# ilovin/lstm_ctc_ocr

Hardware: AMD Instinct MI355X
Metric: captcha images/sec training (32x256, bs=64/GPU) (higher is better)
Workload: dtype bf16; 1 GPU; VGG-7 + BiLSTM(256) + CTC train step, H=32 W=256, 10-char labels, C=64, bs=64/GPU (BASELINE.json configs[1]), Adam lr 1e-4 wd 1e-5 clip 10; global_batch=64, parallelism=dp1, hipgraph=True

## Files before the change

### lstm_ctc_ocr_amd/csrc/common.h

```cpp
#pragma once
#include <stdlib.h>
#include <hip/hip_runtime.h>
#include <stdint.h>
#include <atomic>

#define OCR_WAVE 64

enum {
    OCR_OK = 0,
    OCR_ERR_MEMOPS = 1,
    OCR_ERR_INVALID = 2,
    OCR_ERR_EXEC = 3,
};

#define OCR_CHECK_LAUNCH()                                        \
    do {                                                          \
        hipError_t e__ = hipGetLastError();                       \
        if (e__ != hipSuccess) return OCR_ERR_EXEC;               \
    } while (0)

typedef uint16_t bf16_t;
typedef __attribute__((ext_vector_type(8))) __bf16 bf16x8;
typedef __attribute__((ext_vector_type(4))) float f32x4;
typedef __attribute__((ext_vector_type(4))) unsigned int u32x4;
// ... 3 lines not shown
    uint32_t u = __float_as_uint(f);
    if ((u & 0x7fffffffu) > 0x7f800000u) return (bf16_t)((u >> 16) | 0x40);
    u += 0x7fffu + ((u >> 16) & 1u);
    return (bf16_t)(u >> 16);
}
__device__ __forceinline__ float bf2f(bf16_t h) { return __uint_as_float(((uint32_t)h) << 16); }
typedef __attribute__((ext_vector_type(2))) __bf16 bf16x2_t;
__device__ __forceinline__ uint32_t pack_bf2(float lo, float hi) {
    bf16x2_t v = {(__bf16)lo, (__bf16)hi};
    return __builtin_bit_cast(uint32_t, v);
}
__device__ __forceinline__ float bf_lo(uint32_t p) { return __uint_as_float(p << 16); }
__device__ __forceinline__ float bf_hi(uint32_t p) { return __uint_as_float(p & 0xffff0000u); }

template <int CNT>
__device__ __forceinline__ uint32_t pool_code_word(const u32x4 (&rows)[CNT]) {
    uint32_t word = 0;
#pragma unroll
    for (int c = 0; c < 8; ++c) {
        float v[CNT];
#pragma unroll
        for (int e = 0; e < CNT; ++e) {
            const uint32_t pr = c < 2 ? rows[e].x : c < 4 ? rows[e].y : c < 6 ? rows[e].z : rows[e].w;
            v[e] = (c & 1) ? bf_hi(pr) : bf_lo(pr);
        }
        int best = 0; float bv = v[0];
#pragma unroll
        for (int e = 1; e < CNT; ++e) if (v[e] > bv) { bv = v[e]; best = e; }
        word |= (uint32_t)(best | ((bv > 0.f) ? 4 : 0)) << (4 * c);
    }
    return word;
}

__device__ __forceinline__ float wave_sum(float v) {
#pragma unroll
    for (int o = 32; o > 0; o >>= 1) v += __shfl_xor(v, o, 64);
    return v;
}
__device__ __forceinline__ float wave_max(float v) {
#pragma unroll
    for (int o = 32; o > 0; o >>= 1) v = fmaxf(v, __shfl_xor(v, o, 64));
    return v;
}

__device__ __forceinline__ float sigmoidf_(float x) { return __frcp_rn(1.0f + __expf(-x)); }
__device__ __forceinline__ float tanhf_(float x) {
    float e = __expf(-2.0f * fabsf(x));
    float t = (1.0f - e) * __frcp_rn(1.0f + e);
    return copysignf(t, x);
}

static inline const char* ocr_tune_env(const char* name) {
#ifdef OCR_EXPERIMENTS
    return getenv(name);
#else
    (void)name; return nullptr;
#endif
}
__device__ __forceinline__ long long ocr_wall_clock() { return (long long)__builtin_amdgcn_s_memrealtime(); }
__device__ __forceinline__ void ocr_clk_enter(long long* clk) {
    clk[0] = (long long)__builtin_amdgcn_s_memtime(); clk[1] = ocr_wall_clock();
}
__device__ __forceinline__ void ocr_clk_exit(long long* clk) {
    const long long c = (long long)__builtin_amdgcn_s_memtime(), t = ocr_wall_clock();
    clk[2] = c; clk[3] = t;
    clk[4] += c - clk[0]; clk[5] += t - clk[1]; clk[6] += 1;
// ... 17 lines not shown
```

### lstm_ctc_ocr_amd/csrc/conv_ws.hip

```cpp
#include "conv_plan.h"
#include <type_traits>

enum { WS_BIAS = 1, WS_RELU = 2, WS_MASK = 16, WS_ACCUM = 64 };

struct WsArgs {
    const bf16_t* P; const bf16_t* Q;
    int M, N, C, cW, cH;
    bf16_t* out; const float* bias; const bf16_t* mask; int flags;
    bf16_t* pool; int pool_kind;
    int ntiles, slots, per_slot, xcd_map;
    uint32_t* codes;
};

typedef __attribute__((address_space(3))) void* ws_lptr_t;
#define WS_OOB 0x80000000u

__device__ long long* g_ws_dbg;
extern "C" int ocr_conv_ws_debug(void* dbg) {
    long long* q = (long long*)dbg;
    return hipMemcpyToSymbol(HIP_SYMBOL(g_ws_dbg), &q, sizeof(q)) == hipSuccess ? OCR_OK : OCR_ERR_MEMOPS;
}
#define WS_PHASE(slot) do { if (wsdbg && tid == 0 && (slot) < 64) wsdbg[blockIdx.x * 64 + (slot)] = ocr_wall_clock(); } while (0)
__device__ long long* g_ws_clk;
int ws_set_clock_debug(void* dbg) {
    long long* p = (long long*)dbg;
    return hipMemcpyToSymbol(HIP_SYMBOL(g_ws_clk), &p, sizeof(p)) == hipSuccess ? OCR_OK : OCR_ERR_EXEC;
}

typedef short ws_s16x2 __attribute__((ext_vector_type(2)));
__device__ __forceinline__ uint32_t ws_max2(uint32_t a, uint32_t b) {
    return __builtin_bit_cast(uint32_t, __builtin_elementwise_max(__builtin_bit_cast(ws_s16x2, a), __builtin_bit_cast(ws_s16x2, b)));
}
__device__ __forceinline__ u32x4 ws_max8(u32x4 a, u32x4 b) {
    u32x4 r = {ws_max2(a.x, b.x), ws_max2(a.y, b.y), ws_max2(a.z, b.z), ws_max2(a.w, b.w)};
    return r;
}

typedef unsigned short ws_u16x2 __attribute__((ext_vector_type(2)));
template <int CNT>
__device__ __forceinline__ uint32_t ws_code2(const uint32_t (&p)[CNT]) {
    const ws_u16x2 one = {1, 1};
    ws_u16x2 v[CNT];
#pragma unroll
    for (int e = 0; e < CNT; ++e) v[e] = __builtin_bit_cast(ws_u16x2, p[e]);
    ws_u16x2 m = v[0];
#pragma unroll
    for (int e = 1; e < CNT; ++e) m = __builtin_elementwise_max(m, v[e]);
    ws_u16x2 t = __builtin_elementwise_min((ws_u16x2)(m - v[CNT - 2]), one);
#pragma unroll
    for (int e = CNT - 3; e >= 0; --e) t = __builtin_elementwise_min((ws_u16x2)(m - v[e]), one) * (ws_u16x2)(t + one);
    const ws_u16x2 code = t + (ws_u16x2)(__builtin_elementwise_min(m, one) << (ws_u16x2){2, 2});
    return __builtin_bit_cast(uint32_t, code);
}
template <int CNT>
__device__ __forceinline__ uint32_t ws_code_word(const u32x4 (&p)[CNT]) {
    uint32_t x[CNT], y[CNT], z[CNT], w[CNT];
#pragma unroll
    for (int e = 0; e < CNT; ++e) { x[e] = p[e].x; y[e] = p[e].y; z[e] = p[e].z; w[e] = p[e].w; }
    const uint32_t c0 = ws_code2(x), c1 = ws_code2(y), c2 = ws_code2(z), c3 = ws_code2(w);
    return ((c0 | (c0 >> 12)) & 0xffu) | (((c1 | (c1 >> 12)) & 0xffu) << 8) | (((c2 | (c2 >> 12)) & 0xffu) << 16) | ((c3 | (c3 >> 12)) << 24);
}

template <int H, int NC, int KSPLIT>
struct WsCfg {
    static constexpr int BM = NC * H;
    static constexpr int PG = 4 / KSPLIT;
    static constexpr int CF = NC < 16 ? NC : 16;
    static constexpr int HF = 16 / CF;
    static constexpr int HW = 4 * HF;
    static constexpr int PS = NC + 2;
    static constexpr int CHB = (H + 2) * PS * 128;
    static constexpr int BUFB = KSPLIT * CHB;
    static constexpr int PPC = H * PS / 8;
    static constexpr int PI = KSPLIT * PPC / 4;
    static constexpr int NFE = 4 / KSPLIT;
    static constexpr int HWE = NFE * HF;
    static constexpr int NPE = NC * HWE;
    static constexpr int XOFF = 2 * BUFB;
    static constexpr int SOFF = XOFF + (KSPLIT == 2 ? 4 * 8192 : 0);
    static constexpr int STW = NPE * 128;
    static constexpr int TOFF = SOFF + 4 * STW;
    static constexpr int BOFF = TOFF + 4 * PI * 128;
    static constexpr int MOFF = BOFF + 256;
    static constexpr int LDS_PLAIN = MOFF, LDS_MASK = MOFF + 4 * STW;
    static_assert(((NC + 1) * H + H) * 128 * 2 / 16 * 4 < 65536, "table entries fit 16 bits");
    static_assert(NC == CF && PG * HW == H && (H * PS) % 8 == 0 && (KSPLIT * PPC) % 4 == 0 && LDS_MASK <= 163840, "geometry");
    static_assert(((H + 1) * PS) * 128 < 65536, "ds_read immediates");
};

template <int H, int NC, int KSPLIT, bool MASK ,
          bool CODES = false >
__global__ __launch_bounds__(256) __attribute__((amdgpu_waves_per_eu(1, 1))) void conv_ws_kernel(WsArgs g) {
    using G = WsCfg<H, NC, KSPLIT>;
// ... 325 lines not shown
```

### lstm_ctc_ocr_amd/csrc/nn_ops.hip

```cpp
#include "common.h"
#include <stdlib.h>

__device__ __forceinline__ void unpack8(u32x4 p, float* f) {
    f[0] = bf_lo(p.x); f[1] = bf_hi(p.x); f[2] = bf_lo(p.y); f[3] = bf_hi(p.y);
    f[4] = bf_lo(p.z); f[5] = bf_hi(p.z); f[6] = bf_lo(p.w); f[7] = bf_hi(p.w);
}

__global__ __launch_bounds__(256) void conv1_fwd_kernel(const float* __restrict__ x,
                                                        const float* __restrict__ w,
                                                        const float* __restrict__ bias,
                                                        bf16_t* __restrict__ y, int Nb, int W, int H,
                                                        int Cout, int relu) {
    const int groups = Cout >> 3;
    const int gq = threadIdx.x % groups;
    const int plane = threadIdx.x / groups;
    const int planes = 256 / groups;
    float wr[9][8], br[8];
#pragma unroll
    for (int t = 0; t < 9; ++t)
#pragma unroll
        for (int c = 0; c < 8; ++c) wr[t][c] = w[t * Cout + gq * 8 + c];
#pragma unroll
    for (int c = 0; c < 8; ++c) br[c] = bias[gq * 8 + c];
    const long npix = (long)Nb * W * H;
    for (long pix = (long)blockIdx.x * planes + plane; pix < npix; pix += (long)gridDim.x * planes) {
        int h = (int)(pix % H);
        long q = pix / H;
        int wq = (int)(q % W);
        const float* xn = x + (q - wq) * H;
        float xv[9];
#pragma unroll
        for (int t = 0; t < 9; ++t) {
            int ww = wq + t / 3 - 1, hh = h + t % 3 - 1;
            xv[t] = ((unsigned)ww < (unsigned)W && (unsigned)hh < (unsigned)H) ? xn[(long)ww * H + hh] : 0.f;
// ... 42 lines not shown
#pragma unroll
            for (int c = 0; c < 8; ++c) acc[t][c] = fmaf(xv, dv[c], acc[t][c]);
        }
#pragma unroll
        for (int c = 0; c < 8; ++c) acc[9][c] += dv[c];
    }
    __shared__ float red[4][10][64];
#pragma unroll
    for (int t = 0; t < 10; ++t)
#pragma unroll
        for (int c = 0; c < 8; ++c) {
            float v = acc[t][c];
            v += __shfl_xor(v, 8, 64);
            v += __shfl_xor(v, 16, 64);
            v += __shfl_xor(v, 32, 64);
            acc[t][c] = v;
        }
    const int lane = threadIdx.x & 63, wave = threadIdx.x >> 6;
    if (lane < 8) {
#pragma unroll
        for (int t = 0; t < 10; ++t)
#pragma unroll
            for (int c = 0; c < 8; ++c) red[wave][t][lane * 8 + c] = acc[t][c];
    }
    __syncthreads();
    for (int i = threadIdx.x; i < 10 * 64; i += 256) {
        int t = i / 64, c = i % 64;
        float v = red[0][t][c] + red[1][t][c] + red[2][t][c] + red[3][t][c];
        if (t < 9) atomicAdd(dw + t * Cout + c, v);
        else atomicAdd(db + c, v);
    }
}

__device__ __forceinline__ void conv1_patch(const float* __restrict__ xn, int W, int H, int w0, int h0, float (&patch)[4][4]) {
#pragma unroll
    for (int i = 0; i < 4; ++i)
#pragma unroll
        for (int j = 0; j < 4; ++j) {
            const int ww = w0 - 1 + i, hh = h0 - 1 + j;
            patch[i][j] = ((unsigned)ww < (unsigned)W && (unsigned)hh < (unsigned)H) ? xn[(long)ww * H + hh] : 0.f;
        }
}
__device__ __forceinline__ int conv1_pool_code(float o0, float o1, float o2, float o3) {
    const float r[4] = {bf_lo(pack_bf2(o0, 0.f)), bf_lo(pack_bf2(o1, 0.f)), bf_lo(pack_bf2(o2, 0.f)), bf_lo(pack_bf2(o3, 0.f))};
    int best = 0; float bvv = r[0];
#pragma unroll
    for (int e = 1; e < 4; ++e) if (r[e] > bvv) { bvv = r[e]; best = e; }
    return best | ((bvv > 0.f) ? 4 : 0);
}
__device__ __forceinline__ void conv1_window(const float* __restrict__ xn, int W, int H, int w0, int h0,
                                             const float (&wr)[9][8], const float (&br)[8], float (&o)[4][8], float (&patch)[4][4]) {
    conv1_patch(xn, W, H, w0, h0, patch);
    typedef float f32x2 __attribute__((ext_vector_type(2)));
#pragma unroll
    for (int e = 0; e < 4; ++e) {
        const int a = e >> 1, b = e & 1;
        f32x2 acc2[4];
#pragma unroll
        for (int q = 0; q < 4; ++q) acc2[q] = (f32x2){0.f, 0.f};
#pragma unroll
        for (int t = 0; t < 9; ++t) {
            const float pv = patch[a + t / 3][b + t % 3];
#pragma unroll
            for (int q = 0; q < 4; ++q)
                acc2[q] = __builtin_elementwise_fma((f32x2){pv, pv}, (f32x2){wr[t][2 * q], wr[t][2 * q + 1]}, acc2[q]);
        }
#pragma unroll
        for (int q = 0; q < 4; ++q) {
            o[e][2 * q] = fmaxf(acc2[q].x + br[2 * q], 0.f);
            o[e][2 * q + 1] = fmaxf(acc2[q].y + br[2 * q + 1], 0.f);
        }
    }
}

#ifdef OCR_EXPERIMENTS
struct Conv1Patch { float v[4][4]; };
struct Conv1Raw { float t[4][4]; unsigned ok; };
__device__ __forceinline__ void conv1_patch_load(const float* __restrict__ x, int W, int H, int Wo, int Ho, unsigned op, Conv1Raw& raw) {
    const unsigned ho = op % (unsigned)Ho, q = op / (unsigned)Ho;
    const unsigned wo = q % (unsigned)Wo, n = q / (unsigned)Wo;
    const float* xn = x + (long)n * W * H;
    const int w0 = (int)wo * 2, h0 = (int)ho * 2;
    const bool r0 = w0 > 0, r3 = w0 + 2 < W, c0 = h0 > 0, c3 = h0 + 2 < H;
    const int wi[4] = {r0 ? w0 - 1 : 0, w0, w0 + 1, r3 ? w0 + 2 : w0 + 1};
    const int hj[4] = {c0 ? h0 - 1 : 0, h0, h0 + 1, c3 ? h0 + 2 : h0 + 1};
#pragma unroll
    for (int i = 0; i < 4; ++i)
#pragma unroll
        for (int j = 0; j < 4; ++j) raw.t[i][j] = xn[wi[i] * H + hj[j]];
    raw.ok = (r0 ? 1u : 0u) | (r3 ? 2u : 0u) | (c0 ? 4u : 0u) | (c3 ? 8u : 0u);
}
__device__ __forceinline__ void conv1_patch_select(const Conv1Raw& raw, Conv1Patch& pt) {
    const bool r0 = raw.ok & 1u, r3 = raw.ok & 2u, c0 = raw.ok & 4u, c3 = raw.ok & 8u;
#pragma unroll
    for (int i = 0; i < 4; ++i)
#pragma unroll
        for (int j = 0; j < 4; ++j) {
            const bool ok = (i != 0 || r0) && (i != 3 || r3) && (j != 0 || c0) && (j != 3 || c3);
            pt.v[i][j] = ok ? raw.t[i][j] : 0.f;
        }
}
__device__ __forceinline__ void conv1_pin_weights(float (&wr)[9][8], float (&br)[8]) {
#pragma unroll
    for (int t = 0; t < 9; ++t)
#pragma unroll
        for (int c = 0; c < 8; ++c) asm volatile("" : "+v"(wr[t][c]));
// ... 103 lines not shown
                const float xv = (a == 0) ? ((b == 0) ? cur.v[i][j] : cur.v[i][j + 1]) : ((b == 0) ? cur.v[i + 1][j] : cur.v[i + 1][j + 1]);
                acc[t][c] = fmaf(xv, gv, acc[t][c]);
            }
        }
    }
    __shared__ float red[4][10][64];
#pragma unroll
    for (int t = 0; t < 10; ++t)
#pragma unroll
        for (int c = 0; c < 8; ++c) {
            float v = acc[t][c];
            v += __shfl_xor(v, 8, 64);
            v += __shfl_xor(v, 16, 64);
            v += __shfl_xor(v, 32, 64);
            acc[t][c] = v;
        }
    const int lane = threadIdx.x & 63, wave = threadIdx.x >> 6;
    if (lane < 8) {
#pragma unroll
        for (int t = 0; t < 10; ++t)
#pragma unroll
            for (int c = 0; c < 8; ++c) red[wave][t][lane * 8 + c] = acc[t][c];
    }
    __syncthreads();
    for (int i = threadIdx.x; i < 10 * 64; i += 256) {
        int t = i / 64, c = i % 64;
        float v = red[0][t][c] + red[1][t][c] + red[2][t][c] + red[3][t][c];
        if (t < 9) atomicAdd(dw + t * Cout + c, v);
        else atomicAdd(db + c, v);
    }
}
#endif

template <bool CODES>
__device__ __forceinline__ void conv1_pool_fwd_body(const float* __restrict__ x, const float* __restrict__ w,
                                                    const float* __restrict__ bias, bf16_t* __restrict__ p,
                                                    int Nb, int W, int H, int Cout, f32x4* __restrict__ zero, long zero_n4,
                                                    uint32_t* __restrict__ codes, u32x4* __restrict__ ones, long ones_n4) {
    for (long i = (long)blockIdx.x * 256 + threadIdx.x; i < zero_n4; i += (long)gridDim.x * 256) zero[i] = (f32x4){0.f, 0.f, 0.f, 0.f};
    for (long i = (long)blockIdx.x * 256 + threadIdx.x; i < ones_n4; i += (long)gridDim.x * 256) ones[i] = (u32x4){~0u, ~0u, ~0u, ~0u};
    const int groups = Cout >> 3, gq = threadIdx.x % groups, plane = threadIdx.x / groups, planes = 256 / groups;
    float wr[9][8], br[8];
#pragma unroll
    for (int t = 0; t < 9; ++t)
#pragma unroll
        for (int c = 0; c < 8; ++c) wr[t][c] = w[t * Cout + gq * 8 + c];
#pragma unroll
    for (int c = 0; c < 8; ++c) br[c] = bias[gq * 8 + c];
    const int Wo = W >> 1, Ho = H >> 1;
    const long npix = (long)Nb * Wo * Ho;
    for (long op = (long)blockIdx.x * planes + plane; op < npix; op += (long)gridDim.x * planes) {
        const int ho = (int)(op % Ho);
        const long q = op / Ho;
        const int wo = (int)(q % Wo);
        const long n = q / Wo;
        float o[4][8], patch[4][4];
        conv1_window(x + n * W * H, W, H, wo * 2, ho * 2, wr, br, o, patch);
        float m[8];
#pragma unroll
        for (int c = 0; c < 8; ++c) m[c] = fmaxf(fmaxf(o[0][c], o[1][c]), fmaxf(o[2][c], o[3][c]));
        u32x4 pk = {pack_bf2(m[0], m[1]), pack_bf2(m[2], m[3]), pack_bf2(m[4], m[5]), pack_bf2(m[6], m[7])};
        *(u32x4*)(p + op * Cout + gq * 8) = pk;
        if constexpr (CODES) {
            uint32_t word = 0;
#pragma unroll
            for (int c = 0; c < 8; ++c) word |= (uint32_t)conv1_pool_code(o[0][c], o[1][c], o[2][c], o[3][c]) << (4 * c);
// ... 63 lines not shown
            acc[9][c] += gv;
            const float* px = mypatch + (best >> 1) * 4 + (best & 1);
#pragma unroll
            for (int t = 0; t < 9; ++t) acc[t][c] = fmaf(px[(t / 3) * 4 + t % 3], gv, acc[t][c]);
        }
    }
    __shared__ float red[4][10][64];
#pragma unroll
    for (int t = 0; t < 10; ++t)
#pragma unroll
        for (int c = 0; c < 8; ++c) {
            float v = acc[t][c];
            v += __shfl_xor(v, 8, 64);
            v += __shfl_xor(v, 16, 64);
            v += __shfl_xor(v, 32, 64);
            acc[t][c] = v;
        }
    const int lane = threadIdx.x & 63, wave = threadIdx.x >> 6;
    if (lane < 8) {
#pragma unroll
        for (int t = 0; t < 10; ++t)
#pragma unroll
            for (int c = 0; c < 8; ++c) red[wave][t][lane * 8 + c] = acc[t][c];
    }
    __syncthreads();
    for (int i = threadIdx.x; i < 10 * 64; i += 256) {
        int t = i / 64, c = i % 64;
        float v = red[0][t][c] + red[1][t][c] + red[2][t][c] + red[3][t][c];
        if (slab != nullptr) slab[(long)blockIdx.x * 640 + i] = v;
        else if (t < 9) atomicAdd(dw + t * Cout + c, v);
        else atomicAdd(db + c, v);
    }
}

__device__ __forceinline__ uint32_t max2(uint32_t a, uint32_t b) {
    uint32_t lo = (bf_lo(b) > bf_lo(a)) ? (b & 0xffffu) : (a & 0xffffu);
    uint32_t hi = (bf_hi(b) > bf_hi(a)) ? (b & 0xffff0000u) : (a & 0xffff0000u);
    return lo | hi;
}
__device__ __forceinline__ u32x4 max8(u32x4 a, u32x4 b) {
    u32x4 r = {max2(a.x, b.x), max2(a.y, b.y), max2(a.z, b.z), max2(a.w, b.w)};
    return r;
}

template <int KW, int KH>
__global__ __launch_bounds__(256) void maxpool_fwd_kernel(const bf16_t* __restrict__ x, bf16_t* __restrict__ y,
                                                          int Nb, int W, int H, int C) {
    constexpr int kw = KW, kh = KH;
    const int Wo = W / kw, Ho = H / kh, groups = C >> 3;
    const long total = (long)Nb * Wo * Ho * groups;
    for (long idx = (long)blockIdx.x * 256 + threadIdx.x; idx < total; idx += (long)gridDim.x * 256) {
        int gq = (int)(idx % groups);
        long op = idx / groups;
        int ho = (int)(op % Ho);
        long q = op / Ho;
        int wo = (int)(q % Wo);
        long n = q / Wo;
        const bf16_t* base = x + (((n * W + (long)wo * kw) * H) + (long)ho * kh) * C + gq * 8;
        u32x4 m = *(const u32x4*)base;
#pragma unroll
        for (int a = 0; a < kw; ++a)
#pragma unroll
            for (int b = 0; b < kh; ++b) {
                if (a == 0 && b == 0) continue;
                m = max8(m, *(const u32x4*)(base + ((long)a * H + b) * C));
            }
// ... 772 lines not shown
            const int g = (int)(i / U), u = (int)(i % U);
            out[(u >> 4) * 64 + g * 16 + (u & 15)] = jb.src[i];
        }
    } else {
        for (long i = ((long)b * 256 + threadIdx.x) * 4; i + 3 < jb.n; i += (long)jb.nblocks * 256 * 4) {
            f32x4 v = *(const f32x4*)(jb.src + i);
            u32x2 pk = {pack_bf2(v.x, v.y), pack_bf2(v.z, v.w)};
            *(u32x2*)(jb.dst + i) = pk;
        }
    }
}

__global__ __launch_bounds__(256) void eltwise_bf16_kernel(int op, const bf16_t* __restrict__ a, const bf16_t* __restrict__ b,
                                                           bf16_t* __restrict__ out, long n8) {
    for (long i = (long)blockIdx.x * 256 + threadIdx.x; i < n8; i += (long)gridDim.x * 256) {
        float x[8], y[8], o[8], z[8];
        unpack8(*(const u32x4*)(a + i * 8), x);
        if (op != 1) unpack8(*(const u32x4*)(b + i * 8), y);
        if (op == 4) unpack8(*(const u32x4*)(out + i * 8), z);
#pragma unroll
        for (int c = 0; c < 8; ++c) {
            if (op == 0) o[c] = x[c] + y[c];
            else if (op == 1) o[c] = fmaxf(x[c], 0.f);
            else if (op == 2) o[c] = y[c] > 0.f ? x[c] : 0.f;
            else if (op == 3) o[c] = fmaxf(x[c] + y[c], 0.f);
            else o[c] = z[c] + (y[c] > 0.f ? x[c] : 0.f);
        }
        u32x4 pk = {pack_bf2(o[0], o[1]), pack_bf2(o[2], o[3]), pack_bf2(o[4], o[5]), pack_bf2(o[6], o[7])};
        *(u32x4*)(out + i * 8) = pk;
    }
}

static bool nn_knob(const char* name, int slot) {
    static int v[2] = {-1, -1};
    if (v[slot] < 0) { const char* e = ocr_tune_env(name); v[slot] = (e && atoi(e) != 0) ? 1 : 0; }
    return v[slot] == 1;
}
#ifdef OCR_EXPERIMENTS
static bool conv1_v1() { return !nn_knob("OCR_CONV1_V2", 0); }
#endif
static bool col2im_v1() { return nn_knob("OCR_COL2IM_V1", 1); }
static inline int grid_for(long total, int cap = 4096) {
    long b = (total + 255) / 256;
    if (b > cap) b = cap;
    if (b < 1) b = 1;
    return (int)b;
}

extern "C" int ocr_conv1_fwd(const float* x, const float* w, const float* bias, void* y, int Nb, int W, int H,
                             int Cout, int relu, void* stream) {
    if (!x || !w || !bias || !y || (Cout & 7) || Cout > 1024) return OCR_ERR_INVALID;
    if (256 % (Cout >> 3)) return OCR_ERR_INVALID;
    long total = (long)Nb * W * H * (Cout >> 3);
    conv1_fwd_kernel<<<grid_for(total, 2048), 256, 0, (hipStream_t)stream>>>(
        x, w, bias, (bf16_t*)y, Nb, W, H, Cout, relu);
    OCR_CHECK_LAUNCH();
    return OCR_OK;
}
extern "C" int ocr_conv1_wgrad(const float* x, const void* dz, float* dw, float* db, int Nb, int W, int H, int Cout,
                               void* stream) {
    if (!x || !dz || !dw || !db || Cout != 64) return OCR_ERR_INVALID;
    long npix = (long)Nb * W * H;
    int ppb = 1024;
    conv1_wgrad_kernel<<<ceil_div(npix, ppb), 256, 0, (hipStream_t)stream>>>(x, (const bf16_t*)dz, dw, db, Nb, W, H, Cout, ppb);
    OCR_CHECK_LAUNCH();
    return OCR_OK;
}
extern "C" int ocr_eltwise_bf16(int op, const void* a, const void* b, void* out, long n, void* stream) {
    if (!a || !out || (op != 1 && !b) || op < 0 || op > 4 || n <= 0 || (n & 7)) return OCR_ERR_INVALID;
    eltwise_bf16_kernel<<<grid_for(n / 8, 4096), 256, 0, (hipStream_t)stream>>>(op, (const bf16_t*)a, (const bf16_t*)b, (bf16_t*)out, n / 8);
    OCR_CHECK_LAUNCH();
    return OCR_OK;
}
static int conv1_pool_fwd_impl(const float* x, const float* w, const float* bias, void* p, int Nb, int W, int H, int Cout,
                               float* zero, long zero_n, void* codes, void* ones, long ones_n, void* stream) {
    if (!x || !w || !bias || !p || (Cout & 7) || Cout > 1024 || 256 % (Cout >> 3) || (W & 1) || (H & 1)) return OCR_ERR_INVALID;
    if (zero_n < 0 || (zero_n & 3) || (zero_n && (!zero || ((size_t)zero & 15)))) return OCR_ERR_INVALID;
    if (ones_n < 0 || (ones_n & 3) || (ones_n && (!ones || ((size_t)ones & 15)))) return OCR_ERR_INVALID;
    if (codes && (Cout != 64 || ((size_t)codes & 3))) return OCR_ERR_INVALID;
    long total = (long)Nb * (W / 2) * (H / 2) * (Cout >> 3);
#ifdef OCR_EXPERIMENTS
    if (!zero_n && !ones_n && !codes && !conv1_v1() && (long)Nb * (W / 2) * (H / 2) < 0x7fffffffL && (long)Nb * W * H < 0x7fffffffL && (long)W * H < 0x7fffffffL)
        conv1_pool_fwd2_kernel<<<grid_for(total, 2048), 256, 0, (hipStream_t)stream>>>(x, w, bias, (bf16_t*)p, Nb, W, H, Cout);
    else
#endif
    {
        if (codes) conv1_pool_fwd_kernel<true><<<grid_for(total, 2048), 256, 0, (hipStream_t)stream>>>(x, w, bias, (bf16_t*)p, Nb, W, H, Cout, (f32x4*)zero,
                                                                                                          zero_n / 4, (uint32_t*)codes, (u32x4*)ones, ones_n / 4);
        else conv1_pool_fwd_kernel<false><<<grid_for(total, 2048), 256, 0, (hipStream_t)stream>>>(x, w, bias, (bf16_t*)p, Nb, W, H, Cout, (f32x4*)zero,
                                                                                                 zero_n / 4, nullptr, (u32x4*)ones, ones_n / 4);
    }
    OCR_CHECK_LAUNCH();
    return OCR_OK;
}
extern "C" int ocr_conv1_pool_fwd(const float* x, const float* w, const float* bias, void* p, int Nb, int W, int H, int Cout,
                                  void* stream) {
    return conv1_pool_fwd_impl(x, w, bias, p, Nb, W, H, Cout, nullptr, 0, nullptr, nullptr, 0, stream);
}
extern "C" int ocr_conv1_pool_fwd_train(const float* x, const float* w, const float* bias, void* p, int Nb, int W, int H, int Cout,
                                        void* codes, float* zero, long zero_n, void* ones, long ones_n, void* stream) {
    return conv1_pool_fwd_impl(x, w, bias, p, Nb, W, H, Cout, zero, zero_n, codes, ones, ones_n, stream);
}
static int conv1_ppb() {
    static int v = -1;
    if (v < 0) { const char* e = getenv("OCR_CONV1_PPB"); v = e ? atoi(e) : 256; if (v < 32 || v > 1024 || (v & 31)) v = 256; }
    return v;
}
static int conv1_pool_bwd_impl(const float* x, const float* w, const float* bias, const void* dp, float* dw, float* db,
                               int Nb, int W, int H, int Cout, const void* codes, float* slab, void* stream) {
    if (!x || !w || !bias || !dp || (!slab && (!dw || !db)) || Cout != 64 || (W & 1) || (H & 1) || ((size_t)codes & 3)) return OCR_ERR_INVALID;
    long npix = (long)Nb * (W / 2) * (H / 2);
    int ppb = slab ? conv1_ppb() : 256;
#ifdef OCR_EXPERIMENTS
    if (!codes && !slab && !conv1_v1() && npix < 0x7fffffffL - 512 && (long)Nb * W * H < 0x7fffffffL)
        conv1_pool_bwd2_kernel<<<ceil_div(npix, ppb), 256, 0, (hipStream_t)stream>>>(x, w, bias, (const bf16_t*)dp, dw, db, Nb, W, H,
                                                                                     Cout, ppb);
    else
#endif
    {
        if (codes) conv1_pool_bwd_kernel<true><<<ceil_div(npix, ppb), 256, 0, (hipStream_t)stream>>>(x, w, bias, (const bf16_t*)dp, dw, db, Nb, W, H,
                                                                                                   Cout, ppb, (const uint32_t*)codes, slab);
        else conv1_pool_bwd_kernel<false><<<ceil_div(npix, ppb), 256, 0, (hipStream_t)stream>>>(x, w, bias, (const bf16_t*)dp, dw, db, Nb, W, H,
                                                                                               Cout, ppb, nullptr, slab);
    }
    OCR_CHECK_LAUNCH();
    return OCR_OK;
}
extern "C" int ocr_conv1_pool_bwd(const float* x, const float* w, const float* bias, const void* dp, float* dw, float* db,
                                  int Nb, int W, int H, int Cout, void* stream) {
    return conv1_pool_bwd_impl(x, w, bias, dp, dw, db, Nb, W, H, Cout, nullptr, nullptr, stream);
}
extern "C" int ocr_conv1_pool_bwd_codes(const float* x, const float* w, const float* bias, const void* dp, float* dw, float* db,
                                        int Nb, int W, int H, int Cout, const void* codes, void* stream) {
    if (!codes) return OCR_ERR_INVALID;
    return conv1_pool_bwd_impl(x, w, bias, dp, dw, db, Nb, W, H, Cout, codes, nullptr, stream);
}
extern "C" int ocr_conv1_pool_bwd_slab_rows(int Nb, int W, int H) {
    if (Nb <= 0 || W <= 0 || H <= 0 || (W & 1) || (H & 1)) return 0;
    return (int)ceil_div((long)Nb * (W / 2) * (H / 2), (long)conv1_ppb());
}
extern "C" int ocr_conv1_pool_bwd_slab(const float* x, const float* w, const float* bias, const void* dp, int Nb, int W, int H, int Cout,
                                       const void* codes, float* slab, void* stream) {
    if (!slab || ((size_t)slab & 15)) return OCR_ERR_INVALID;
    return conv1_pool_bwd_impl(x, w, bias, dp, nullptr, nullptr, Nb, W, H, Cout, codes, slab, stream);
}
extern "C" int ocr_maxpool_fwd(const void* x, void* y, int Nb, int W, int H, int C, int kw, int kh, void* stream) {
    if (!x || !y || (C & 7) || kw < 1 || kw > 2 || kh < 1 || kh > 2 || W % kw || H % kh) return OCR_ERR_INVALID;
    long total = (long)Nb * (W / kw) * (H / kh) * (C >> 3);
    const bf16_t* xi = (const bf16_t*)x; bf16_t* yo = (bf16_t*)y;
    hipStream_t st = (hipStream_t)stream;
    int gr = grid_for(total, 8192);
    if (kw == 2 && kh == 2) maxpool_fwd_kernel<2, 2><<<gr, 256, 0, st>>>(xi, yo, Nb, W, H, C);
    else if (kw == 1 && kh == 2) maxpool_fwd_kernel<1, 2><<<gr, 256, 0, st>>>(xi, yo, Nb, W, H, C);
    else if (kw == 2 && kh == 1) maxpool_fwd_kernel<2, 1><<<gr, 256, 0, st>>>(xi, yo, Nb, W, H, C);
    else return OCR_ERR_INVALID;
    OCR_CHECK_LAUNCH();
    return OCR_OK;
// ... 272 lines not shown
```

Before: 56360 images/sec.

## Stage conv1 input rows in LDS tiles for fused conv+pool forward and backward

Replaces the default conv1+maxpool forward and backward kernels with tile kernels. Each block stages the contiguous span of input rows it needs into shared memory, with zero padding, then computes per-pixel 3x3 windows from LDS instead of global loads. Index divisions are replaced by precomputed reciprocal multiplies. The forward pass packs bf16 outputs and pool codes with a shared u16 max/code helper, and the old kernels stay reachable only under experiment knobs. This trades global-memory traffic for dynamic LDS allocation that may limit occupancy, and adds new geometry checks that return an error on large shapes.

```diff
diff --git a/lstm_ctc_ocr_amd/csrc/common.h b/lstm_ctc_ocr_amd/csrc/common.h
--- a/lstm_ctc_ocr_amd/csrc/common.h
+++ b/lstm_ctc_ocr_amd/csrc/common.h
@@ -59,6 +59,27 @@
     return word;
 }
 
+typedef unsigned short u16x2_t __attribute__((ext_vector_type(2)));
+template <int CNT>
+__device__ __forceinline__ uint32_t pool_code2_u16(const uint32_t (&p)[CNT], uint32_t& mx) {
+    const u16x2_t one = {1, 1};
+    u16x2_t v[CNT];
+#pragma unroll
+    for (int e = 0; e < CNT; ++e) v[e] = __builtin_bit_cast(u16x2_t, p[e]);
+    u16x2_t m = v[0];
+#pragma unroll
+    for (int e = 1; e < CNT; ++e) m = __builtin_elementwise_max(m, v[e]);
+    u16x2_t t = __builtin_elementwise_min((u16x2_t)(m - v[CNT - 2]), one);
+#pragma unroll
+    for (int e = CNT - 3; e >= 0; --e) t = __builtin_elementwise_min((u16x2_t)(m - v[e]), one) * (u16x2_t)(t + one);
+    const u16x2_t code = t + (u16x2_t)(__builtin_elementwise_min(m, one) << (u16x2_t){2, 2});
+    mx = __builtin_bit_cast(uint32_t, m);
+    return __builtin_bit_cast(uint32_t, code);
+}
+__device__ __forceinline__ uint32_t pool_code2_merge(uint32_t c0, uint32_t c1, uint32_t c2, uint32_t c3) {
+    return ((c0 | (c0 >> 12)) & 0xffu) | (((c1 | (c1 >> 12)) & 0xffu) << 8) | (((c2 | (c2 >> 12)) & 0xffu) << 16) | ((c3 | (c3 >> 12)) << 24);
+}
+
 __device__ __forceinline__ float wave_sum(float v) {
 #pragma unroll
     for (int o = 32; o > 0; o >>= 1) v += __shfl_xor(v, o, 64);
diff --git a/lstm_ctc_ocr_amd/csrc/conv_ws.hip b/lstm_ctc_ocr_amd/csrc/conv_ws.hip
--- a/lstm_ctc_ocr_amd/csrc/conv_ws.hip
+++ b/lstm_ctc_ocr_amd/csrc/conv_ws.hip
@@ -36,21 +36,10 @@
     return r;
 }
 
-typedef unsigned short ws_u16x2 __attribute__((ext_vector_type(2)));
 template <int CNT>
 __device__ __forceinline__ uint32_t ws_code2(const uint32_t (&p)[CNT]) {
-    const ws_u16x2 one = {1, 1};
-    ws_u16x2 v[CNT];
-#pragma unroll
-    for (int e = 0; e < CNT; ++e) v[e] = __builtin_bit_cast(ws_u16x2, p[e]);
-    ws_u16x2 m = v[0];
-#pragma unroll
-    for (int e = 1; e < CNT; ++e) m = __builtin_elementwise_max(m, v[e]);
-    ws_u16x2 t = __builtin_elementwise_min((ws_u16x2)(m - v[CNT - 2]), one);
-#pragma unroll
-    for (int e = CNT - 3; e >= 0; --e) t = __builtin_elementwise_min((ws_u16x2)(m - v[e]), one) * (ws_u16x2)(t + one);
-    const ws_u16x2 code = t + (ws_u16x2)(__builtin_elementwise_min(m, one) << (ws_u16x2){2, 2});
-    return __builtin_bit_cast(uint32_t, code);
+    uint32_t mx;
+    return pool_code2_u16(p, mx);
 }
 template <int CNT>
 __device__ __forceinline__ uint32_t ws_code_word(const u32x4 (&p)[CNT]) {
@@ -58,7 +47,7 @@
 #pragma unroll
     for (int e = 0; e < CNT; ++e) { x[e] = p[e].x; y[e] = p[e].y; z[e] = p[e].z; w[e] = p[e].w; }
     const uint32_t c0 = ws_code2(x), c1 = ws_code2(y), c2 = ws_code2(z), c3 = ws_code2(w);
-    return ((c0 | (c0 >> 12)) & 0xffu) | (((c1 | (c1 >> 12)) & 0xffu) << 8) | (((c2 | (c2 >> 12)) & 0xffu) << 16) | ((c3 | (c3 >> 12)) << 24);
+    return pool_code2_merge(c0, c1, c2, c3);
 }
 
 template <int H, int NC, int KSPLIT>
diff --git a/lstm_ctc_ocr_amd/csrc/nn_ops.hip b/lstm_ctc_ocr_amd/csrc/nn_ops.hip
--- a/lstm_ctc_ocr_amd/csrc/nn_ops.hip
+++ b/lstm_ctc_ocr_amd/csrc/nn_ops.hip
@@ -1,5 +1,6 @@
 #include "common.h"
 #include <stdlib.h>
+#include <algorithm>
 
 __device__ __forceinline__ void unpack8(u32x4 p, float* f) {
     f[0] = bf_lo(p.x); f[1] = bf_hi(p.x); f[2] = bf_lo(p.y); f[3] = bf_hi(p.y);
@@ -108,6 +109,30 @@
     }
 }
 
+__device__ __forceinline__ void conv1_window_fma(const float (&patch)[4][4], const float (&wr)[9][8], const float (&br)[8], float (&o)[4][8]) {
+    typedef float f32x2 __attribute__((ext_vector_type(2)));
+#pragma unroll
+    for (int e = 0; e < 4; ++e) {
+        const int a = e >> 1, b = e & 1;
+        f32x2 acc2[4];
+#pragma unroll
+        for (int q = 0; q < 4; ++q) acc2[q] = (f32x2){0.f, 0.f};
+#pragma unroll
+        for (int t = 0; t < 9; ++t) {
+            const float pv = patch[a + t / 3][b + t % 3];
+#pragma unroll
+            for (int q = 0; q < 4; ++q)
+                acc2[q] = __builtin_elementwise_fma((f32x2){pv, pv}, (f32x2){wr[t][2 * q], wr[t][2 * q + 1]}, acc2[q]);
+        }
+#pragma unroll
+        for (int q = 0; q < 4; ++q) {
+            o[e][2 * q] = fmaxf(acc2[q].x + br[2 * q], 0.f);
+            o[e][2 * q + 1] = fmaxf(acc2[q].y + br[2 * q + 1], 0.f);
+        }
+    }
+}
+
+#ifdef OCR_EXPERIMENTS
 __device__ __forceinline__ void conv1_patch(const float* __restrict__ xn, int W, int H, int w0, int h0, float (&patch)[4][4]) {
 #pragma unroll
     for (int i = 0; i < 4; ++i)
@@ -127,27 +152,9 @@
 __device__ __forceinline__ void conv1_window(const float* __restrict__ xn, int W, int H, int w0, int h0,
                                              const float (&wr)[9][8], const float (&br)[8], float (&o)[4][8], float (&patch)[4][4]) {
     conv1_patch(xn, W, H, w0, h0, patch);
-    typedef float f32x2 __attribute__((ext_vector_type(2)));
-#pragma unroll
-    for (int e = 0; e < 4; ++e) {
-        const int a = e >> 1, b = e & 1;
-        f32x2 acc2[4];
-#pragma unroll
-        for (int q = 0; q < 4; ++q) acc2[q] = (f32x2){0.f, 0.f};
-#pragma unroll
-        for (int t = 0; t < 9; ++t) {
-            const float pv = patch[a + t / 3][b + t % 3];
-#pragma unroll
-            for (int q = 0; q < 4; ++q)
-                acc2[q] = __builtin_elementwise_fma((f32x2){pv, pv}, (f32x2){wr[t][2 * q], wr[t][2 * q + 1]}, acc2[q]);
-        }
-#pragma unroll
-        for (int q = 0; q < 4; ++q) {
-            o[e][2 * q] = fmaxf(acc2[q].x + br[2 * q], 0.f);
-            o[e][2 * q + 1] = fmaxf(acc2[q].y + br[2 * q + 1], 0.f);
-        }
-    }
-}
+    conv1_window_fma(patch, wr, br, o);
+}
+#endif
 
 #ifdef OCR_EXPERIMENTS
 struct Conv1Patch { float v[4][4]; };
@@ -317,6 +324,7 @@
 }
 #endif
 
+#ifdef OCR_EXPERIMENTS
 template <bool CODES>
 __device__ __forceinline__ void conv1_pool_fwd_body(const float* __restrict__ x, const float* __restrict__ w,
                                                     const float* __restrict__ bias, bf16_t* __restrict__ p,
@@ -446,6 +454,198 @@
         else atomicAdd(db + c, v);
     }
 }
+#endif
+
+struct Conv1Geo { int RS, Ho, Wo; unsigned ho0, wo0, rHo, rWo; };
+__device__ __forceinline__ unsigned conv1_div(unsigned v, unsigned r) { return r ? __umulhi(v, r) : v; }
+__device__ __forceinline__ Conv1Geo conv1_tile_stage(const float* __restrict__ x, int Nb, int W, int H, unsigned p0, unsigned p1, unsigned rH,
+                                                     unsigned rHo, unsigned rWo, float* __restrict__ tile) {
+    Conv1Geo g;
+    g.RS = H + 2; g.Ho = H >> 1; g.Wo = W >> 1; g.rHo = rHo; g.rWo = rWo;
+    const unsigned q0 = p0 / (unsigned)g.Ho, q1 = (p1 - 1) / (unsigned)g.Ho;
+    g.ho0 = p0 - q0 * (unsigned)g.Ho; g.wo0 = q0 % (unsigned)g.Wo;
+    const int rows = 2 * (int)(q1 - q0 + 1) + 2;
+    const long first = (2 * (long)q0 - 1) * H, total = (long)Nb * W * H;
+    for (unsigned i = threadIdx.x; i < (unsigned)(rows * H); i += 256) {
+        const unsigned r = __umulhi(i, rH), h = i - r * (unsigned)H;
+        const long e = first + i;
+        tile[r * g.RS + 1 + h] = (e >= 0 && e < total) ? x[e] : 0.f;
+    }
+    for (int r = threadIdx.x; r < rows; r += 256) { tile[r * g.RS] = 0.f; tile[r * g.RS + H + 1] = 0.f; }
+    __syncthreads();
+    return g;
+}
+struct Conv1Pix { const float* base; bool top, bottom; };
+__device__ __forceinline__ Conv1Pix conv1_tile_pixel(const float* __restrict__ tile, const Conv1Geo& g, unsigned i) {
+    const unsigned v = g.ho0 + i, qi = conv1_div(v, g.rHo), ho = v - qi * (unsigned)g.Ho;
+    const unsigned c = g.wo0 + qi, wo = c - conv1_div(c, g.rWo) * (unsigned)g.Wo;
+    Conv1Pix px = {tile + (2 * qi) * g.RS + 2 * ho, wo == 0, wo == (unsigned)g.Wo - 1};
+    return px;
+}
+__device__ __forceinline__ void conv1_tile_patch(const Conv1Pix& px, int RS, float (&patch)[4][4]) {
+#pragma unroll
+    for (int a = 0; a < 4; ++a)
+#pragma unroll
+        for (int b = 0; b < 4; ++b) patch[a][b] = px.base[a * RS + b];
+#pragma unroll
+    for (int b = 0; b < 4; ++b) { patch[0][b] = px.top ? 0.f : patch[0][b]; patch[3][b] = px.bottom ? 0.f : patch[3][b]; }
+}
+__device__ __forceinline__ uint32_t conv1_pool_pack(const float (&o)[4][8], u32x4& pk) {
+    uint32_t m[4], cd[4];
+#pragma unroll
+    for (int q = 0; q < 4; ++q) {
+        uint32_t pe[4];
+#pragma unroll
+        for (int e = 0; e < 4; ++e) {
+            typedef float f32x2 __attribute__((ext_vector_type(2)));
+            pe[e] = __builtin_bit_cast(uint32_t, __builtin_convertvector((f32x2){o[e][2 * q], o[e][2 * q + 1]}, bf16x2_t));
+        }
+        cd[q] = pool_code2_u16(pe, m[q]);
+    }
+    pk = (u32x4){m[0], m[1], m[2], m[3]};
+    return pool_code2_merge(cd[0], cd[1], cd[2], cd[3]);
+}
+
+template <bool CODES>
+__global__ __launch_bounds__(256) void conv1_pool_fwd_tile_kernel(const float* __restrict__ x, const float* __restrict__ w, const float* __restrict__ bias,
+                                                                  bf16_t* __restrict__ p, int Nb, int W, int H, int Cout, int pix_per_block, unsigned rH,
+                                                                  unsigned rHo, unsigned rWo, f32x4* __restrict__ zero, long zero_n4,
+                                                                  uint32_t* __restrict__ codes, u32x4* __restrict__ ones, long ones_n4) {
+    extern __shared__ float conv1_tile[];
+    for (long i = (long)blockIdx.x * 256 + threadIdx.x; i < zero_n4; i += (long)gridDim.x * 256) zero[i] = (f32x4){0.f, 0.f, 0.f, 0.f};
+    for (long i = (long)blockIdx.x * 256 + threadIdx.x; i < ones_n4; i += (long)gridDim.x * 256) ones[i] = (u32x4){~0u, ~0u, ~0u, ~0u};
+    const unsigned npix = (unsigned)Nb * (W >> 1) * (H >> 1);
+    const unsigned p0 = blockIdx.x * (unsigned)pix_per_block, p1 = min(npix, p0 + (unsigned)pix_per_block);
+    if (p0 >= npix) return;
+    const int groups = Cout >> 3, gq = threadIdx.x % groups, plane = threadIdx.x / groups, planes = 256 / groups;
+    float wr[9][8], br[8];
+#pragma unroll
+    for (int t = 0; t < 9; ++t)
+#pragma unroll
+        for (int c = 0; c < 8; ++c) wr[t][c] = w[t * Cout + gq * 8 + c];
+#pragma unroll
+    for (int c = 0; c < 8; ++c) br[c] = bias[gq * 8 + c];
+    const Conv1Geo geo = conv1_tile_stage(x, Nb, W, H, p0, p1, rH, rHo, rWo, conv1_tile);
+    for (unsigned i = plane; i < p1 - p0; i += planes) {
+        float o[4][8], patch[4][4];
+        conv1_tile_patch(conv1_tile_pixel(conv1_tile, geo, i), geo.RS, patch);
+        conv1_window_fma(patch, wr, br, o);
+        u32x4 pk;
+        const uint32_t word = conv1_pool_pack(o, pk);
+        const long op = (long)p0 + i;
+        *(u32x4*)(p + op * Cout + gq * 8) = pk;
+        if constexpr (CODES) codes[op * groups + gq] = word;
+    }
+}
+
+__device__ __forceinline__ void conv1_bwd_reduce(float (&acc)[10][8], float* __restrict__ dw, float* __restrict__ db, float* __restrict__ slab) {
+    __shared__ float red[4][10][64];
+#pragma unroll
+    for (int t = 0; t < 10; ++t)
+#pragma unroll
+        for (int c = 0; c < 8; ++c) {
+            float v = acc[t][c];
+            v += __shfl_xor(v, 8, 64);
+            v += __shfl_xor(v, 16, 64);
+            v += __shfl_xor(v, 32, 64);
+            acc[t][c] = v;
+        }
+    const int lane = threadIdx.x & 63, wave = threadIdx.x >> 6;
+    if (lane < 8) {
+#pragma unroll
+        for (int t = 0; t < 10; ++t)
+#pragma unroll
+            for (int c = 0; c < 8; ++c) red[wave][t][lane * 8 + c] = acc[t][c];
+    }
+    __syncthreads();
+    for (int i = threadIdx.x; i < 10 * 64; i += 256) {
+        int t = i / 64, c = i % 64;
+        float v = red[0][t][c] + red[1][t][c] + red[2][t][c] + red[3][t][c];
+        if (slab != nullptr) slab[(long)blockIdx.x * 640 + i] = v;
+        else if (t < 9) atomicAdd(dw + t * 64 + c, v);
+        else atomicAdd(db + c, v);
+    }
+}
+
+template <bool CODES , bool LOOKUP>
+__global__ __launch_bounds__(256) void conv1_pool_bwd_tile_kernel(const float* __restrict__ x, const float* __restrict__ w, const float* __restrict__ bias,
+                                                                  const bf16_t* __restrict__ dp, float* __restrict__ dw, float* __restrict__ db, int Nb,
+                                                                  int W, int H, int pix_per_block, unsigned rH, unsigned rHo, unsigned rWo,
+                                                                  const uint32_t* __restrict__ codes, float* __restrict__ slab) {
+    extern __shared__ float conv1_tile[];
+    typedef float f32x2 __attribute__((ext_vector_type(2)));
+    const int gq = threadIdx.x & 7, pl = threadIdx.x >> 3;
+    float wr[CODES ? 1 : 9][8], br[8];
+    if (!CODES) {
+#pragma unroll
+        for (int t = 0; t < 9; ++t)
+#pragma unroll
+            for (int c = 0; c < 8; ++c) wr[CODES ? 0 : t][c] = w[t * 64 + gq * 8 + c];
+#pragma unroll
+        for (int c = 0; c < 8; ++c) br[c] = bias[gq * 8 + c];
+    }
+    const unsigned npix = (unsigned)Nb * (W >> 1) * (H >> 1);
+    const unsigned p0 = blockIdx.x * (unsigned)pix_per_block, p1 = min(npix, p0 + (unsigned)pix_per_block);
+    f32x2 acc2[10][4];
+#pragma unroll
+    for (int t = 0; t < 10; ++t)
+#pragma unroll
+        for (int q = 0; q < 4; ++q) acc2[t][q] = (f32x2){0.f, 0.f};
+    const Conv1Geo geo = conv1_tile_stage(x, Nb, W, H, p0, p1, rH, rHo, rWo, conv1_tile);
+    for (unsigned i = pl; i < p1 - p0; i += 32) {
+        const long op = (long)p0 + i;
+        float patch[4][4];
+        uint32_t word = 0;
+        const Conv1Pix px = conv1_tile_pixel(conv1_tile, geo, i);
+        conv1_tile_patch(px, geo.RS, patch);
+        if constexpr (CODES) {
+            word = codes[op * 8 + gq];
+        } else {
+            float o[4][8];
+            u32x4 pk;
+            conv1_window_fma(patch, wr, br, o);
+            word = conv1_pool_pack(o, pk);
+        }
+        float g[8];
+        unpack8(*(const u32x4*)(dp + op * 64 + gq * 8), g);
+#pragma unroll
+        for (int q = 0; q < 4; ++q) {
+            const int c0 = (int)((word >> (8 * q)) & 7u), c1 = (int)((word >> (8 * q + 4)) & 7u);
+            const f32x2 gv = {(c0 & 4) ? g[2 * q] : 0.f, (c1 & 4) ? g[2 * q + 1] : 0.f};
+            acc2[9][q] += gv;
+            if constexpr (LOOKUP) {
+                const int a0 = c0 >> 1 & 1, a1 = c1 >> 1 & 1;
+                const float* t0 = px.base + a0 * geo.RS + (c0 & 1);
+                const float* t1 = px.base + a1 * geo.RS + (c1 & 1);
+                const bool zt0 = px.top && !a0, zb0 = px.bottom && a0, zt1 = px.top && !a1, zb1 = px.bottom && a1;
+#pragma unroll
+                for (int t = 0; t < 9; ++t) {
+                    f32x2 xv = {t0[(t / 3) * geo.RS + t % 3], t1[(t / 3) * geo.RS + t % 3]};
+                    if (t / 3 == 0) xv = (f32x2){zt0 ? 0.f : xv.x, zt1 ? 0.f : xv.y};
+                    if (t / 3 == 2) xv = (f32x2){zb0 ? 0.f : xv.x, zb1 ? 0.f : xv.y};
+                    acc2[t][q] = __builtin_elementwise_fma(xv, gv, acc2[t][q]);
+                }
+            } else {
+#pragma unroll
+                for (int e = 0; e < 4; ++e) {
+                    const f32x2 ge = {(c0 & 3) == e ? gv.x : 0.f, (c1 & 3) == e ? gv.y : 0.f};
+#pragma unroll
+                    for (int t = 0; t < 9; ++t) {
+                        const float pv = patch[(e >> 1) + t / 3][(e & 1) + t % 3];
+                        acc2[t][q] = __builtin_elementwise_fma((f32x2){pv, pv}, ge, acc2[t][q]);
+                    }
+                }
+            }
+        }
+    }
+    float acc[10][8];
+#pragma unroll
+    for (int t = 0; t < 10; ++t)
+#pragma unroll
+        for (int q = 0; q < 4; ++q) { acc[t][2 * q] = acc2[t][q].x; acc[t][2 * q + 1] = acc2[t][q].y; }
+    conv1_bwd_reduce(acc, dw, db, slab);
+}
+
 
 __device__ __forceinline__ uint32_t max2(uint32_t a, uint32_t b) {
     uint32_t lo = (bf_lo(b) > bf_lo(a)) ? (b & 0xffffu) : (a & 0xffffu);
@@ -1284,12 +1484,14 @@
 }
 
 static bool nn_knob(const char* name, int slot) {
-    static int v[2] = {-1, -1};
+    static int v[4] = {-1, -1, -1, -1};
     if (v[slot] < 0) { const char* e = ocr_tune_env(name); v[slot] = (e && atoi(e) != 0) ? 1 : 0; }
     return v[slot] == 1;
 }
 #ifdef OCR_EXPERIMENTS
 static bool conv1_v1() { return !nn_knob("OCR_CONV1_V2", 0); }
+static bool conv1_gen1() { return nn_knob("OCR_CONV1_GEN", 2); }
+static bool conv1_lookup() { return nn_knob("OCR_CONV1_LOOKUP", 3); }
 #endif
 static bool col2im_v1() { return nn_knob("OCR_COL2IM_V1", 1); }
 static inline int grid_for(long total, int cap = 4096) {
@@ -1324,6 +1526,24 @@
     OCR_CHECK_LAUNCH();
     return OCR_OK;
 }
+struct Conv1Launch { bool ok; int blocks, ppb, lds; unsigned rH, rHo, rWo; };
+static unsigned conv1_recip(long d) { return d > 1 ? (unsigned)((0x100000000ull + (unsigned long)d - 1) / (unsigned long)d) : 0u; }
+static Conv1Launch conv1_launch(int Nb, int W, int H, int ppb) {
+    Conv1Launch L = {};
+    if (Nb < 0 || W < 2 || H < 2) return L;
+    const long Wo = W / 2, Ho = H / 2, npix = (long)Nb * Wo * Ho;
+    const long cols = std::min<long>(2 + (ppb - 1) / Ho, std::max<long>((long)Nb * Wo, 1)), words = (2 * cols + 2) * (H + 2);
+    if (npix >= 0x7fffffffL || words * 4 > 160 * 1024) return L;
+    if ((Ho + ppb) * Ho >= 0x100000000L || (Wo + cols) * Wo >= 0x100000000L || words * H >= 0x100000000L) return L;
+    L.ok = true; L.ppb = ppb; L.blocks = std::max(1, ceil_div(npix, ppb)); L.lds = (int)words * 4;
+    L.rH = conv1_recip(H); L.rHo = conv1_recip(Ho); L.rWo = conv1_recip(Wo);
+    return L;
+}
+static int conv1_fwd_ppb() {
+    static int v = -1;
+    if (v < 0) { const char* e = ocr_tune_env("OCR_CONV1_FWD_PPB"); v = e ? atoi(e) : 128; if (v < 32 || v > 1024 || (v & 31)) v = 128; }
+    return v;
+}
 static int conv1_pool_fwd_impl(const float* x, const float* w, const float* bias, void* p, int Nb, int W, int H, int Cout,
                                float* zero, long zero_n, void* codes, void* ones, long ones_n, void* stream) {
     if (!x || !w || !bias || !p || (Cout & 7) || Cout > 1024 || 256 % (Cout >> 3) || (W & 1) || (H & 1)) return OCR_ERR_INVALID;
@@ -1331,16 +1551,26 @@
     if (ones_n < 0 || (ones_n & 3) || (ones_n && (!ones || ((size_t)ones & 15)))) return OCR_ERR_INVALID;
     if (codes && (Cout != 64 || ((size_t)codes & 3))) return OCR_ERR_INVALID;
     long total = (long)Nb * (W / 2) * (H / 2) * (Cout >> 3);
+    const Conv1Launch L = conv1_launch(Nb, W, H, conv1_fwd_ppb());
+    if (!L.ok) return OCR_ERR_INVALID;
 #ifdef OCR_EXPERIMENTS
     if (!zero_n && !ones_n && !codes && !conv1_v1() && (long)Nb * (W / 2) * (H / 2) < 0x7fffffffL && (long)Nb * W * H < 0x7fffffffL && (long)W * H < 0x7fffffffL)
         conv1_pool_fwd2_kernel<<<grid_for(total, 2048), 256, 0, (hipStream_t)stream>>>(x, w, bias, (bf16_t*)p, Nb, W, H, Cout);
-    else
-#endif
-    {
+    else if (conv1_gen1()) {
         if (codes) conv1_pool_fwd_kernel<true><<<grid_for(total, 2048), 256, 0, (hipStream_t)stream>>>(x, w, bias, (bf16_t*)p, Nb, W, H, Cout, (f32x4*)zero,
                                                                                                           zero_n / 4, (uint32_t*)codes, (u32x4*)ones, ones_n / 4);
         else conv1_pool_fwd_kernel<false><<<grid_for(total, 2048), 256, 0, (hipStream_t)stream>>>(x, w, bias, (bf16_t*)p, Nb, W, H, Cout, (f32x4*)zero,
                                                                                                  zero_n / 4, nullptr, (u32x4*)ones, ones_n / 4);
+    } else
+#endif
+    if (codes) {
+        if (ocr_allow_lds<conv1_pool_fwd_tile_kernel<true>>(L.lds) != hipSuccess) return OCR_ERR_EXEC;
+        conv1_pool_fwd_tile_kernel<true><<<L.blocks, 256, L.lds, (hipStream_t)stream>>>(x, w, bias, (bf16_t*)p, Nb, W, H, Cout, L.ppb, L.rH, L.rHo, L.rWo,
+                                                                                       (f32x4*)zero, zero_n / 4, (uint32_t*)codes, (u32x4*)ones, ones_n / 4);
+    } else {
+        if (ocr_allow_lds<conv1_pool_fwd_tile_kernel<false>>(L.lds) != hipSuccess) return OCR_ERR_EXEC;
+        conv1_pool_fwd_tile_kernel<false><<<L.blocks, 256, L.lds, (hipStream_t)stream>>>(x, w, bias, (bf16_t*)p, Nb, W, H, Cout, L.ppb, L.rH, L.rHo, L.rWo,
+                                                                                        (f32x4*)zero, zero_n / 4, nullptr, (u32x4*)ones, ones_n / 4);
     }
     OCR_CHECK_LAUNCH();
     return OCR_OK;
@@ -1358,23 +1588,33 @@
     if (v < 0) { const char* e = getenv("OCR_CONV1_PPB"); v = e ? atoi(e) : 256; if (v < 32 || v > 1024 || (v & 31)) v = 256; }
     return v;
 }
+#define CONV1_BWD_TILE(CODES, LOOKUP)                                                                                              \
+    do {                                                                                                                           \
+        if (ocr_allow_lds<conv1_pool_bwd_tile_kernel<CODES, LOOKUP>>(L.lds) != hipSuccess) return OCR_ERR_EXEC;                    \
+        conv1_pool_bwd_tile_kernel<CODES, LOOKUP><<<nb, 256, L.lds, (hipStream_t)stream>>>(x, w, bias, g, dw, db, Nb, W, H, ppb,    \
+                                                                                            L.rH, L.rHo, L.rWo, cd, slab);         \
+    } while (0)
 static int conv1_pool_bwd_impl(const float* x, const float* w, const float* bias, const void* dp, float* dw, float* db,
                                int Nb, int W, int H, int Cout, const void* codes, float* slab, void* stream) {
     if (!x || !w || !bias || !dp || (!slab && (!dw || !db)) || Cout != 64 || (W & 1) || (H & 1) || ((size_t)codes & 3)) return OCR_ERR_INVALID;
     long npix = (long)Nb * (W / 2) * (H / 2);
     int ppb = slab ? conv1_ppb() : 256;
+    const Conv1Launch L = conv1_launch(Nb, W, H, ppb);
+    if (!L.ok) return OCR_ERR_INVALID;
+    const bf16_t* g = (const bf16_t*)dp;
+    const uint32_t* cd = (const uint32_t*)codes;
+    const int nb = ceil_div(npix, ppb);
 #ifdef OCR_EXPERIMENTS
     if (!codes && !slab && !conv1_v1() && npix < 0x7fffffffL - 512 && (long)Nb * W * H < 0x7fffffffL)
-        conv1_pool_bwd2_kernel<<<ceil_div(npix, ppb), 256, 0, (hipStream_t)stream>>>(x, w, bias, (const bf16_t*)dp, dw, db, Nb, W, H,
-                                                                                     Cout, ppb);
-    else
+        conv1_pool_bwd2_kernel<<<nb, 256, 0, (hipStream_t)stream>>>(x, w, bias, g, dw, db, Nb, W, H, Cout, ppb);
+    else if (conv1_gen1()) {
+        if (codes) conv1_pool_bwd_kernel<true><<<nb, 256, 0, (hipStream_t)stream>>>(x, w, bias, g, dw, db, Nb, W, H, Cout, ppb, cd, slab);
+        else conv1_pool_bwd_kernel<false><<<nb, 256, 0, (hipStream_t)stream>>>(x, w, bias, g, dw, db, Nb, W, H, Cout, ppb, nullptr, slab);
+    } else if (conv1_lookup()) {
+        if (codes) CONV1_BWD_TILE(true, true); else CONV1_BWD_TILE(false, true);
+    } else
 #endif
-    {
-        if (codes) conv1_pool_bwd_kernel<true><<<ceil_div(npix, ppb), 256, 0, (hipStream_t)stream>>>(x, w, bias, (const bf16_t*)dp, dw, db, Nb, W, H,
-                                                                                                   Cout, ppb, (const uint32_t*)codes, slab);
-        else conv1_pool_bwd_kernel<false><<<ceil_div(npix, ppb), 256, 0, (hipStream_t)stream>>>(x, w, bias, (const bf16_t*)dp, dw, db, Nb, W, H,
-                                                                                               Cout, ppb, nullptr, slab);
-    }
+    if (codes) CONV1_BWD_TILE(true, false); else CONV1_BWD_TILE(false, false);
     OCR_CHECK_LAUNCH();
     return OCR_OK;
 }
```

Measured after the change: 56940 images/sec (median of 6 runs). 1.0% higher.
